# Psy-Fer/SquiggleKit

Hardware: AMD Instinct MI355X
Metric: reads/sec MotifSeq DTW (4k-sample read x 200-sample motif) (higher is better)
Workload: dtype f64 results; u32 fixed-point screening

## Files before the change

### squigglekit_amd/csrc/sk_api.hip

```cpp
#include "sk_common.h"
#include <math.h>
#include <string.h>
#include <stdio.h>
#include <stdlib.h>
#include <vector>

namespace {

int check_i16(const void *sig, int64_t stride, const int32_t *len, int32_t nreads)
{
    if (nreads < 0) return sk_fail(SK_ERR_INVALID, "nreads < 0");
    if (nreads && (!sig || !len)) return sk_fail(SK_ERR_INVALID, "NULL sig/len");
    if (stride <= 0) return sk_fail(SK_ERR_INVALID, "stride must be positive");
    return SK_OK;
}

int check_len_host(const int32_t *len, int32_t nreads, int64_t stride)
{
    for (int32_t r = 0; r < nreads; r++)
        if (len[r] < 0 || (int64_t)len[r] > stride)
            return sk_fail(SK_ERR_INVALID, "len[%d] = %d is outside [0, stride = %lld]", r, len[r], (long long)stride);
    return SK_OK;
}

// ... 42 lines not shown
    cost[0] = fabs(x[0] - y[0]);
    for (int i = 1; i < n; i++) cost[(size_t)i * m] = fabs(x[i] - y[0]) + cost[(size_t)(i - 1) * m];
    for (int j = 1; j < m; j++) cost[j] = fabs(x[0] - y[j]);
    for (int i = 1; i < n; i++) {
        const double *up = cost + (size_t)(i - 1) * m;
        double *row = cost + (size_t)i * m;
        for (int j = 1; j < m; j++) row[j] = fabs(x[i] - y[j]) + cref_min3(up[j], up[j - 1], row[j - 1]);
    }
    const double *last = cost + (size_t)(n - 1) * m;
    int idx = 0;
    double best = last[0];
    if (!(best != best))
        for (int j = 1; j < m; j++) {
            if (last[j] != last[j]) { idx = j; break; }
            if (last[j] < best) { best = last[j]; idx = j; }
        }
    int i = n - 1, j = idx;
    while (i > 0) {
        if (j == 0) { i--; continue; }
        const double up = cost[(size_t)(i - 1) * m + j], dg = cost[(size_t)(i - 1) * m + j - 1], lf = cost[(size_t)i * m + j - 1];
        const double mc = cref_min3(up, dg, lf);
        if (dg == mc)      { i--; j--; }
        else if (lf == mc) { j--; }
        else               { i--; }
    }
    sk_hit h;
    h.dist = last[idx]; h.start = j; h.end = idx; h.n = m; h.flags = 0;
    out[0] = h;
}

struct SubBatches {
    int32_t per = 0, n = 1;
};
SubBatches sub_batches(int32_t nreads, int64_t stride)
{
    SubBatches sb;
    int64_t target = (int64_t)256 << 20;
    if (const char *e = sk_tune("SK_INGEST_MB")) { const long v = atol(e); if (v > 0) target = (int64_t)v << 20; }
    int64_t per = target / (stride * (int64_t)sizeof(int16_t));
    if (per < 4096) per = 4096;
    if (per * 2 > nreads) { sb.per = nreads; sb.n = 1; return sb; }
    sb.n = (int32_t)((nreads + per - 1) / per);
    sb.per = (int32_t)(((int64_t)nreads + sb.n - 1) / sb.n);
    return sb;
}

template <class Step>
int ingest_rows(sk_ctx *c, const SubBatches &B, int16_t *d_rows, const int16_t *sig, int64_t stride, const int32_t *len,
                int32_t nreads, Step step)
{
    int rc;
    if (B.n > 1 && (rc = sk_second_stream(c))) return rc;
    const hipStream_t cs = B.n > 1 ? c->stream2 : c->stream;
    for (int32_t bi = 0; bi < B.n; bi++) {
        const int32_t r0 = bi * B.per;
        const int32_t nr = (nreads - r0 < B.per) ? nreads - r0 : B.per;
        if (nr <= 0) break;
        int16_t *d_sig = d_rows + (size_t)r0 * (size_t)stride;
        int32_t *d_len = (int32_t *)c->len.p + r0;
        SK_HIP(hipMemcpyAsync(d_sig, sig + (size_t)r0 * (size_t)stride, (size_t)nr * (size_t)stride * sizeof(int16_t),
                              hipMemcpyHostToDevice, cs));
        if (len) SK_HIP(hipMemcpyAsync(d_len, len + r0, (size_t)nr * sizeof(int32_t), hipMemcpyHostToDevice, cs));
        if (B.n > 1) {
            SK_HIP(hipEventRecord(c->ev_chunk[bi & 7], cs));
            SK_HIP(hipStreamWaitEvent(c->stream, c->ev_chunk[bi & 7], 0));
        }
        if ((rc = step(r0, nr, d_sig, d_len))) return rc;
    }
    return SK_OK;
}

void redo_forget(sk_ctx *c)
{
    c->redo_route = SK_REDO_NONE;
    c->redo_off.clear();
    c->redo_used = 0;
}

int redo_begin(sk_ctx *c, int32_t nreads, int32_t lists)
{
    redo_forget(c);
    return sk_reserve(c, &c->redo, ((size_t)nreads + 16 * (size_t)lists) * sizeof(int32_t));
}

int redo_list(sk_ctx *c, int route, int32_t nr, int32_t **list)
{
    const size_t end = c->redo_used + (size_t)nr + 16;
    if (end * sizeof(int32_t) > c->redo.cap) return sk_fail(SK_ERR_INVALID, "internal: redo list past its reservation");
    *list = (int32_t *)c->redo.p + c->redo_used;
    c->redo_used = end;
    c->redo_route = route;
    return SK_OK;
}

int redo_count(sk_ctx *c, int route)
{
    if (c->redo_route != route) return -1;
    SK_HIP(hipStreamSynchronize(c->stream));
    int total = 0;
    for (size_t o : c->redo_off) {
        int32_t v = 0;
        SK_HIP(hipMemcpy(&v, (const int32_t *)c->redo.p + o, sizeof v, hipMemcpyDeviceToHost));
        total += v;
    }
    return total;
}
// ... 2388 lines not shown
```

### squigglekit_amd/csrc/sk_common.h

```cpp
#pragma once
#include <hip/hip_runtime.h>
#include <stdint.h>
#include <stddef.h>
#include <stdarg.h>
#include <vector>
#include "squigglekit_hip.h"

#define SK_MAX_DEVICES 16
#define SK_WAVE 64

struct sk_prep {
    int32_t n;
    int32_t flags;
    double  center;
    double  scale;
    double  top;
    double  bot;
};

#define SK_IFLAG_INPLACE 0x100
#define SK_FLAG_PUBLIC   0xff

enum sk_prep_mode { SK_PREP_MEDMAD = 0, SK_PREP_ZSCALE = 1, SK_PREP_SEGMENT = 2, SK_PREP_DRNA = 3 };

enum sk_redo_route { SK_REDO_NONE = 0, SK_REDO_I16 = 1, SK_REDO_F64 = 2, SK_REDO_PA = 3 };

struct sk_buf {
    void  *p = nullptr;
    size_t cap = 0;
};

struct sk_panel_motif {
    int32_t xoff;
    int32_t P;
    int32_t k;
    int32_t pad;
};
struct sk_panel_group {
    int32_t L, R;
    int32_t first, count;
};

struct sk_ctx {
    int         device = -1;
    bool        ready = false;
    hipStream_t stream = nullptr;
    hipStream_t stream2 = nullptr;
    hipStream_t stream3 = nullptr;
    hipEvent_t  ev_r[2] = {nullptr, nullptr};
    hipStream_t stream4 = nullptr;
    hipEvent_t  ev_a = nullptr;
    hipEvent_t  ev_s[2] = {nullptr, nullptr};
    uint32_t    dtw_sparse_calls = 0;
    uint32_t    dtw_audit_calls = 0;
    hipEvent_t  ev_chunk[9] = {};
    hipEvent_t  ev[4] = {nullptr, nullptr, nullptr, nullptr};
    bool        ev_valid = false;
    int         num_cu = 0;
    sk_buf sig;
    sk_buf len;
    sk_buf rlen;
    sk_buf off;
    sk_buf comp;
    sk_buf prep;
    sk_buf mask;
    sk_buf motif;
    sk_buf out;
    sk_buf out2;
    sk_buf misc;
    sk_buf seghints;
    sk_buf pacal;
    sk_buf pull;
    sk_buf pulltext;
    sk_buf sweep;
    sk_buf sweeprec;
    sk_buf hitrows;
    sk_buf bgrec;
    sk_buf pathcnt;
    bool   path_valid = false;
    sk_buf pathlist;
    sk_buf pathscratch;
    sk_buf pathmotif;
    sk_buf pathspans;
    sk_buf events;
    sk_buf poolev;
    sk_buf pool;
    sk_buf panel;
    sk_buf panelwin;
    sk_buf panelaux;
    sk_buf panelrec;
    sk_buf seglev;
    sk_buf seglevwork;
    sk_buf detect;
    sk_buf detectout;
    sk_buf hmm;
    sk_buf hmmpath;
    sk_buf hmmseg;
    std::vector<double> panel_host;
    std::vector<sk_panel_motif> panel_table;
    std::vector<sk_panel_group> panel_groups;
    std::vector<int32_t> panel_long;
    sk_buf ckpt;
    sk_buf motifq;
    sk_buf motif64;
    bool   motif64_valid = false;
    std::vector<double> motif64_host;
    sk_buf lastq;
    sk_buf qflag;
    sk_buf wsoft;
    sk_buf lsum;
    sk_buf wstate;
    sk_buf wrec;
    sk_buf wrecq;
    sk_buf order;
    sk_buf motifw;
    std::vector<double> motifw_host;
    int    motifq_L = 0;
    sk_buf retry;
    sk_buf dtwcnt;
    sk_buf audit;
    sk_buf sib;
    sk_buf sibout;
    sk_buf sibstate;
    bool   retry_dev = false;
    std::vector<unsigned> motifq_host;
    bool   motifq_valid = false;
    sk_buf redo;
    int    redo_route = SK_REDO_NONE;
    std::vector<size_t> redo_off;
    size_t redo_used = 0;
    std::vector<int64_t> pa_off_host;
    int    last_retry = 0;
    std::vector<hipEvent_t> evpool;
    int    prof_chunks = 0;
    int    prof_reads[64] = {0};
    std::vector<double> motif_host;
    std::vector<double> motif_src;
    int    motif_L = 0;
    void  *comm = nullptr;
    sk_buf commbuf;
};

const char *sk_tune(const char *name);

struct sk_entry {
    sk_ctx *c = nullptr;
    sk_entry();
    explicit sk_entry(int slot);
    ~sk_entry();
    sk_entry(const sk_entry &) = delete;
    sk_entry &operator=(const sk_entry &) = delete;
};
#define SK_ENTER(c)                                                                     \
    sk_entry c##_entry_;                                                                \
    sk_ctx *const c = c##_entry_.c;                                                     \
    if (!c) return SK_ERR_NO_DEVICE
sk_ctx *sk_ctx_of(int device);
int  sk_bound_device(void);
int  sk_fail(int code, const char *fmt, ...);
int  sk_reserve(sk_ctx *c, sk_buf *b, size_t bytes);
int  sk_second_stream(sk_ctx *c);
int64_t sk_dtw_chunk_reads(size_t per_read, int64_t nreads);
void    sk_dtw_scratch_shrink(int reset);
#define SK_HIP(call)                                                                    \
    do {                                                                                \
        hipError_t e_ = (call);                                                         \
        if (e_ != hipSuccess)                                                           \
            return sk_fail(SK_ERR_HIP, "%s failed: %s (%s:%d)", #call,                 \
                           hipGetErrorString(e_), __FILE__, __LINE__);                  \
    } while (0)

int sk_launch_prep_i16(sk_ctx *c, const int16_t *d_sig, int64_t stride, const int32_t *d_len,
                       int32_t nreads, int32_t lo, int32_t hi, int mode, double std_scale,
                       int16_t *d_comp, sk_prep *d_prep, uint64_t *d_mask, int64_t mask_stride,
                       int32_t t0 = 0, int32_t t1 = 0x7fffffff,
                       const int32_t *d_list = nullptr, const int32_t *d_count = nullptr,
// ... 197 lines not shown
```

### squigglekit_amd/csrc/sk_runtime.hip

```cpp
#include "sk_common.h"
#include <string>
#include <string.h>
#include <mutex>
#include <stdio.h>
#include <stdlib.h>
#include <string.h>

static thread_local char  g_err[512] = "";
static thread_local int   g_cur = -1;
static sk_ctx             g_ctx[SK_MAX_DEVICES];
static std::mutex         g_mu;
static std::recursive_mutex g_ctx_mu[SK_MAX_DEVICES];

int sk_fail(int code, const char *fmt, ...)
{
    va_list ap;
    va_start(ap, fmt);
    vsnprintf(g_err, sizeof g_err, fmt, ap);
    va_end(ap);
    return code;
}

sk_entry::sk_entry() : sk_entry(g_cur) {}

// ... 9 lines not shown
            return;
        }
        g_ctx_mu[slot].unlock();
    }
    sk_fail(SK_ERR_NO_DEVICE, "no device bound: call sk_init(device) first (no CPU fallback exists)");
}

sk_entry::~sk_entry() { if (c) g_ctx_mu[c - g_ctx].unlock(); }

sk_ctx *sk_ctx_of(int device) { return (device >= 0 && device < SK_MAX_DEVICES) ? &g_ctx[device] : nullptr; }
int sk_bound_device(void) { return g_cur; }

int sk_reserve(sk_ctx *c, sk_buf *b, size_t bytes)
{
    (void)c;
    if (bytes <= b->cap) return SK_OK;
    if (b->p) { SK_HIP(hipFree(b->p)); b->p = nullptr; b->cap = 0; }
    size_t want = bytes + bytes / 8 + 256;
    hipError_t e = hipMalloc(&b->p, want);
    if (e != hipSuccess) {
        b->p = nullptr;
        return sk_fail(SK_ERR_NOMEM, "hipMalloc(%zu) failed: %s", want, hipGetErrorString(e));
    }
    b->cap = want;
    return SK_OK;
}

int sk_second_stream(sk_ctx *c)
{
    if (!c->stream2) {
        SK_HIP(hipStreamCreateWithFlags(&c->stream2, hipStreamNonBlocking));
        for (int i = 0; i < 9; i++) SK_HIP(hipEventCreateWithFlags(&c->ev_chunk[i], hipEventDisableTiming));
    }
    return SK_OK;
}

struct sk_tunable { const char *name, *test_values, *what; };
static const sk_tunable SK_TUNABLES[] = {
    {"SK_DTW_SCHEME",         "full exact2", "DTW scheme: full = one exact pass, exact2 = two exact passes (default: fixed-point screening + certified window)"},
    {"SK_DTW_QL",             "8 16 64",     "lanes per read of the screening scheme (default: by motif length and batch size)"},
    {"SK_DTW_NOFUSE",         "1",           "filter + medmad as their own kernel instead of the screening pass's prologue"},
    {"SK_DTW_FORCE_RETRY_PM", "100 1000",    "per-mille of reads sent through the exact retry whatever the window pass certified (sensitivity runs)"},
    {"SK_DTW_SPAN",           "150 300",     "look-back of the window pass in columns (one tier)"},
    {"SK_DTW_SPAN2",          "0 500",       "look-back of the window pass's second tier (0: none)"},
    {"SK_DTW_CK",             "64 256",      "steps between checkpoints of the screening pass (multiple of 64)"},
    {"SK_DTW_NOSORT",         "1",           "window passes take the reads in file order"},
    {"SK_DTW_SORT_MIN",       "1",           "window passes sort chunks of at least this many reads"},
    {"SK_DTW_NO_EARLY",       "1",           "no early exact retry beside the window passes"},
    {"SK_DTW_NO_SIBLINGS",    "1",           "reads whose candidate columns fall into two clusters take the exact pass (no second window)"},
    {"SK_DTW_NOGUARD",        "1",           "screening scheme without its run-time guard (premise test in the window pass, audit, gated exact fallback): A/B cost runs"},
    {"SK_DTW_AUDIT_PERIOD",   "0 1 64",      "the audit re-runs one read in this many with the exact pass (default 4096; 0: no audit)"},
    {"SK_DTW_HOLE",           "qerr1 fma64 fma64x", "tests: a known precision hole put back (E = 1; the fma sample image for float64 reads, with / without the image-error guard) -- the guard has to notice and the records must not change"},
    {"SK_DTW_SCRATCH_MB",     "8 64",        "checkpoint scratch budget in MB (small values force many chunks)"},
    {"SK_DTW_NO_SMALL",       "1",           "small batches keep the batch lane layout"},
    {"SK_DTW_SMALL_MAX",      "0 100000",    "largest batch that spreads a read over 64 lanes"},
    {"SK_PREP_BLOCK",         "1",           "medmad statistics by the workgroup-per-read kernel"},
    {"SK_PREP_ROUNDS",        "1 3",         "grid rounds of the persistent statistics kernels"},
    {"SK_PREP_PERCU",         "1 2",         "workgroups per CU of the persistent statistics kernels"},
    {"SK_SEG_OLD",            "1",           "segmenter: numpy-order statistics kernels for every read"},
    {"SK_SEG_DELTA_SCALE",    "1e13",        "segmenter: certification margin multiplier (large: every read takes the numpy-order redo)"},
    {"SK_SEG_PA_F64",         "1",           "segmenter, raw reads through the pA conversion: expand to float64 and take the float64 kernels instead of the raw-domain kernel"},
    {"SK_SEG_NO_WG",          "1",           "segmenter, reads of 4 097 .. 65 536 samples: the wavefront-per-read statistics kernel (two looks at a read) instead of the workgroup-per-read one"},
    {"SK_SEG_WG_ALL",         "1",           "segmenter: the workgroup-per-read statistics kernel for every row of 4 097 .. 65 536 samples (default: where it is faster)"},
    {"SK_SEG_OCC",            "7 8",         "segmenter statistics kernel: waves per SIMD the registers are sized for"},
    {"SK_SEG_CHUNKS",         "2 8",         "segmenter: chunks of a large batch (walk of one beside the statistics of the next)"},
    {"SK_WALK_GENERAL",       "1",           "segmenter walk: general step (corrector test live)"},
    {"SK_WALK_SYNC",          "1",           "segmenter walk: run hopping with the 64 lanes of a wavefront on the same word (k_seg_walk3)"},
    {"SK_WALK_OWNPASS",       "1",           "segmenter walk: finds the quiet stretches and anchors in a pass of its own instead of taking the statistics kernel's hints"},
    {"SK_WALK_NOJUMP",        "1",           "segmenter walk: every run is hopped through, no jumps between the stretches of quiet entries"},
    {"SK_WALK_NOWAVE",        "1",           "segmenter walk: a lane per read also for long rows / small batches (no wavefront-per-read walk)"},
    {"SK_WALK_WAVE_MAXREADS", "0 1000000",   "segmenter walk: batches of up to this many reads take the wavefront-per-read walk (default: 16384, 131072 for rows beyond 4 096 samples)"},
    {"SK_DRNA_STEP",          "1",           "dRNA_segmenter, both branches: the per-sample scans instead of the scans by runs / by transitions"},
    {"SK_ROLL_TWO_KERNELS",   "1",           "dRNA_segmenter rolling-mean branch: filter kernel + prefix sums through HBM instead of the one-look kernel (prefix sums in LDS)"},
    {"SK_ROLL_ONE_LOOK",      "1",           "dRNA_segmenter rolling-mean branch: the workgroup-per-read kernel in numpy's order for every read instead of the streaming kernel with certified thresholds"},
    {"SK_ROLL_DELTA_SCALE",   "1e13",        "dRNA_segmenter rolling-mean branch: multiplier of the certification margin (large: every read is redone in numpy's order)"},
    {"SK_HITS_ROW_BYTES",     "1000000",     "hit lists: bytes of the last-row buffer (12 B per column and read; default 2 GiB; small values force many chunks of reads)"},
    {"SK_PANEL_EXACT",        "1",           "motif panel: the one-grid exact kernel also for long windows over many reads (default: those take the screening scheme, one launch set per motif)"},
    {"SK_PATH_LDS_BYTES",     "0",           "alignment paths: bytes of direction words a hit may keep in LDS (default and most 25600; 0: every hit takes the scratch tier)"},
    {"SK_PATH_SCRATCH_BYTES", "1000000",     "alignment paths: byte budget of the scratch tier's slabs (default 1 GiB; small values leave one wavefront)"},
    {"SK_INGEST_MB",          "1 4",         "sub-batch size of the host entry points in MB"},
    {"SK_HMM_SCRATCH_MB",     "1",           "signal HMM state paths: back-pointer scratch budget in MB (default 16384; small values force slices of one 64-read group)"},
    {"SK_F64_OLD",            "1",           "float64 reads: numpy-order statistics kernel for every read"},
    {"SK_F64_LONG_LOOKS",     "1",           "float64 reads of 4 097 .. 40 960 samples: the window-by-window kernel (three to five looks at a read) instead of the workgroup-per-read one (one look)"},
};

const char *sk_tune(const char *name)
{
    const char *on = getenv("SK_TUNING");
    if (!on || on[0] != '1') return nullptr;
    for (const sk_tunable &t : SK_TUNABLES)
        if (strcmp(t.name, name) == 0) return getenv(name);
    return nullptr;
}

static thread_local int g_dtw_shrink = 0;
void sk_dtw_scratch_shrink(int reset) { g_dtw_shrink = reset ? 0 : (g_dtw_shrink < 12 ? g_dtw_shrink + 1 : 12); }

int64_t sk_dtw_chunk_reads(size_t per_read, int64_t nreads)
{
    size_t budget = (size_t)64 << 30;
    int64_t floor_reads = 1024;
    if (const char *e = sk_tune("SK_DTW_SCRATCH_MB")) {
        const long v = atol(e);
        if (v > 0) { budget = (size_t)v << 20; floor_reads = 64; }
    }
    budget >>= g_dtw_shrink;
// ... 24 lines not shown
        sk_fail(SK_ERR_NO_DEVICE, "hipGetDeviceCount: %s", hipGetErrorString(e));
        return 0;
    }
    return n;
}

int sk_init(int device) { return sk_init_slot(device, device); }

int sk_init_slot(int slot, int device)
{
    int n = sk_device_count();
    if (n <= 0) return sk_fail(SK_ERR_NO_DEVICE, "no HIP device visible (this library has no CPU fallback)");
    if (device < 0 || device >= n || device >= SK_MAX_DEVICES)
        return sk_fail(SK_ERR_INVALID, "device %d out of range (0..%d)", device, n - 1);
    if (slot < 0 || slot >= SK_MAX_DEVICES)
        return sk_fail(SK_ERR_INVALID, "context slot %d out of range (0..%d)", slot, SK_MAX_DEVICES - 1);
    std::lock_guard<std::mutex> lk(g_mu);
    sk_ctx *c = &g_ctx[slot];
    std::lock_guard<std::recursive_mutex> c_lock(g_ctx_mu[slot]);
    if (c->ready && c->device != device)
        return sk_fail(SK_ERR_INVALID, "context slot %d already serves device %d", slot, c->device);
    SK_HIP(hipSetDevice(device));
    if (!c->ready) {
        hipDeviceProp_t prop;
        SK_HIP(hipGetDeviceProperties(&prop, device));
        if (strncmp(prop.gcnArchName, "gfx950", 6) != 0)
            return sk_fail(SK_ERR_NO_DEVICE, "device %d is %s; this build targets gfx950 only",
                           device, prop.gcnArchName);
        c->device = device;
        c->num_cu = prop.multiProcessorCount;
        SK_HIP(hipStreamCreateWithFlags(&c->stream, hipStreamNonBlocking));
        for (int i = 0; i < 4; i++) SK_HIP(hipEventCreate(&c->ev[i]));
        c->ready = true;
    }
    g_cur = slot;
    return SK_OK;
}

static void free_buf(sk_buf *b) { if (b->p) (void)hipFree(b->p); b->p = nullptr; b->cap = 0; }

int sk_shutdown(void)
{
    std::lock_guard<std::mutex> lk(g_mu);
    for (int d = 0; d < SK_MAX_DEVICES; d++) {
        sk_ctx *c = &g_ctx[d];
        std::lock_guard<std::recursive_mutex> c_lock(g_ctx_mu[d]);
        if (!c->ready) continue;
        (void)hipSetDevice(c->device);
        (void)hipStreamSynchronize(c->stream);
        sk_buf *bufs[] = {&c->sig, &c->len, &c->off, &c->comp, &c->prep, &c->mask,
                          &c->motif, &c->out, &c->out2, &c->misc, &c->ckpt, &c->retry, &c->motifq, &c->lastq, &c->qflag,
                          &c->motif64, &c->commbuf, &c->dtwcnt, &c->wsoft, &c->wstate, &c->wrec, &c->motifw, &c->lsum, &c->wrecq, &c->order, &c->pacal, &c->seghints, &c->audit, &c->rlen, &c->redo, &c->sib, &c->sibout, &c->sibstate, &c->pull, &c->pulltext, &c->sweep, &c->sweeprec, &c->hitrows, &c->bgrec, &c->pathcnt, &c->pathlist, &c->pathscratch, &c->pathmotif, &c->pathspans, &c->events, &c->poolev, &c->pool, &c->panel, &c->panelwin, &c->panelaux, &c->panelrec, &c->seglev, &c->seglevwork, &c->detect, &c->detectout, &c->hmm, &c->hmmpath, &c->hmmseg};
        for (sk_buf *b : bufs) free_buf(b);
        for (int i = 0; i < 4; i++) (void)hipEventDestroy(c->ev[i]);
        for (hipEvent_t e : c->evpool) (void)hipEventDestroy(e);
        if (c->stream2) {
            (void)hipStreamSynchronize(c->stream2);
            for (int i = 0; i < 9; i++) if (c->ev_chunk[i]) (void)hipEventDestroy(c->ev_chunk[i]);
            (void)hipStreamDestroy(c->stream2);
        }
        if (c->stream3) {
            (void)hipStreamSynchronize(c->stream3);
            for (int i = 0; i < 2; i++) if (c->ev_r[i]) (void)hipEventDestroy(c->ev_r[i]);
            (void)hipStreamDestroy(c->stream3);
        }
        for (int i = 0; i < 2; i++) if (c->ev_s[i]) (void)hipEventDestroy(c->ev_s[i]);
        if (c->stream4) {
            (void)hipStreamSynchronize(c->stream4);
            if (c->ev_a) (void)hipEventDestroy(c->ev_a);
            (void)hipStreamDestroy(c->stream4);
        }
        (void)hipStreamDestroy(c->stream);
        *c = sk_ctx();
    }
    g_cur = -1;
    return SK_OK;
}

int sk_sync(void)
{
    SK_ENTER(c);
    SK_HIP(hipStreamSynchronize(c->stream));
    return SK_OK;
}

int sk_device_name(char *buf, int cap)
{
    SK_ENTER(c);
    if (!buf || cap <= 0) return sk_fail(SK_ERR_INVALID, "bad buffer");
    hipDeviceProp_t prop;
    SK_HIP(hipGetDeviceProperties(&prop, c->device));
    snprintf(buf, (size_t)cap, "%s (%s, %d CUs)", prop.name, prop.gcnArchName, prop.multiProcessorCount);
    return SK_OK;
}

int sk_device_pci_bus_id(char *buf, int cap)
{
    SK_ENTER(c);
    if (!buf || cap < 16) return sk_fail(SK_ERR_INVALID, "bad buffer");
    SK_HIP(hipDeviceGetPCIBusId(buf, cap, c->device));
    return SK_OK;
}

void *sk_dev_alloc(size_t bytes)
{
    sk_entry entry;
// ... 149 lines not shown
```

### squigglekit_amd/csrc/sk_sdtw.hip

```cpp
#include "sk_sdtw_dev.h"
#include <math.h>
#include <stdlib.h>
#include <string.h>
#include <vector>

namespace {

template <int L, int R, int FEED, int MODE>
__global__ __launch_bounds__(256)
void k_sdtw(const sdtw_kargs a)
{
    static_assert(L == 16 || L == 64, "lanes per read");
    constexpr int G = 64 / L;
    constexpr int SHR = (L == 16) ? DPP_ROW_SHR1 : DPP_WAVE_SHR1;
    constexpr int ROL = (L == 16) ? DPP_ROW_ROL1 : DPP_WAVE_ROL1;
    constexpr bool TRACK = (MODE != MODE_DIST);
    constexpr int CKW = R + 3;
    const double INF = __builtin_huge_val();

    const int lane = threadIdx.x & 63;
    const int wave = blockIdx.x * (blockDim.x >> 6) + (threadIdx.x >> 6);
    const int g = lane / L, l = lane % L;
    int slot = wave * G + g;
    int nreads = a.nreads;
// ... 580 lines not shown
    int32_t *alist = nullptr;  sk_hit *aout = nullptr;
    if (naudit) {
        if ((rc = sk_reserve(c, &c->audit, ((size_t)naudit + 2) * sizeof(int32_t) + 16 + (size_t)naudit * sizeof(sk_hit)))) return rc;
        alist = (int32_t *)c->audit.p;
        aout = (sk_hit *)((char *)c->audit.p + ((((size_t)naudit + 2) * sizeof(int32_t) + 15) & ~(size_t)15));
    }
    auto launch_audit = [&](hipStream_t stream) -> int {
        if (!naudit) return SK_OK;
        sk_audit_pick(alist, naudit, audit_period, a->nreads, c->dtw_audit_calls++, stream ? stream : c->stream);
        SK_HIP(hipGetLastError());
        sdtw_kargs kr = k;
        kr.read0 = 0; kr.ridx = alist + 2; kr.count_ptr = alist; kr.ckpt = nullptr; kr.out = aout; kr.out_by_slot = 1;
        kr.total_ptr = guard + SK_GUARD_AUDITED; kr.list_off = 0;
        const int R64 = (N + 63) / 64, P64 = 64 * R64 - N;
        sdtw_fn f64 = (L == 16) ? pick_any(a->feed, 64, R64, MODE_FULL) : nullptr;
        if (f64) {
            sdtw_kargs k64 = kr;
            k64.xlay = (const double *)c->motif64.p; k64.P = P64;
            k64.nreads = naudit < 8192 ? naudit : 8192;
            int rc2;
            if ((rc2 = launch(c, f64, k64, 64, stream))) return rc2;
            if (naudit <= 8192) return SK_OK;
            kr.list_off = 8192; kr.total_ptr = nullptr; kr.nreads = naudit - 8192;
            return launch(c, ff, kr, L, stream);
        }
        kr.nreads = naudit;
        return launch(c, ff, kr, L, stream);
    };
    auto finish_guard = [&]() -> int {
        if (!guarded) return SK_OK;
        if (naudit) {
            sk_audit_compare(alist, aout, a->out, naudit, guard, c->stream);
            SK_HIP(hipGetLastError());
        }
        sdtw_kargs kf = k;
        kf.read0 = 0; kf.nreads = a->nreads; kf.ridx = nullptr; kf.count_ptr = nullptr; kf.ckpt = nullptr;
        kf.gate_ptr = guard + SK_GUARD_ALARM; kf.guard = guard;
        return launch(c, ff, kf, L);
    };
    if (qok) {
        const bool early = sk_tune("SK_DTW_NO_EARLY") == nullptr;
        if (early && !c->stream3) {
            SK_HIP(hipStreamCreateWithFlags(&c->stream3, hipStreamNonBlocking));
            for (int i = 0; i < 2; i++) SK_HIP(hipEventCreateWithFlags(&c->ev_r[i], hipEventDisableTiming));
        }
        if (early && naudit && !c->stream4) {
            SK_HIP(hipStreamCreateWithFlags(&c->stream4, hipStreamNonBlocking));
            SK_HIP(hipEventCreateWithFlags(&c->ev_a, hipEventDisableTiming));
        }
        if ((rc = sk_launch_sdtw_screen(c, a, ck, span_q, span2, cnt, cnt + 2, early ? ecnt : nullptr,
                                        early ? ecnt + 2 : nullptr))) return rc;
        if (early) {
            SK_HIP(hipStreamWaitEvent(c->stream3, c->ev_r[0], 0));
            if ((rc = launch_retry(ecnt, c->stream3))) return rc;
            SK_HIP(hipEventRecord(c->ev_r[1], c->stream3));
            if (naudit) {
                SK_HIP(hipStreamWaitEvent(c->stream4, c->ev_r[0], 0));
                if ((rc = launch_audit(c->stream4))) return rc;
                SK_HIP(hipEventRecord(c->ev_a, c->stream4));
            }
        }
        if ((rc = launch_retry())) return rc;
        if (early) {
            SK_HIP(hipStreamWaitEvent(c->stream, c->ev_r[1], 0));
            if (naudit) SK_HIP(hipStreamWaitEvent(c->stream, c->ev_a, 0));
        } else if ((rc = launch_audit(nullptr))) return rc;
        if ((rc = finish_guard())) return rc;
        SK_HIP(hipEventRecord(c->ev[3], c->stream));
        return SK_OK;
    }
    const int nck = (int)((maxlen + L - 1) / ck);
    const size_t per_read = (size_t)(nck > 0 ? nck : 1) * L * (R + 3) * sizeof(double);
    int64_t chunk;
    while (true) {
        chunk = sk_dtw_chunk_reads(per_read, a->nreads);
        rc = sk_reserve(c, &c->ckpt, (size_t)chunk * per_read);
        if (rc != SK_ERR_NOMEM || chunk <= 1024) break;
        sk_dtw_scratch_shrink(0);
    }
    if (rc) return rc;
    k.ckpt = (double *)c->ckpt.p; k.nck = nck; k.ck = ck; k.span = span;
    k.retry = cnt + 2; k.retry_cnt = cnt;
    const size_t nchunks = (size_t)((a->nreads + chunk - 1) / chunk);
    while (c->evpool.size() < 3 * nchunks) {
        hipEvent_t e;
        SK_HIP(hipEventCreate(&e));
        c->evpool.push_back(e);
    }
    c->prof_chunks = 0;
    for (int64_t r0 = 0; r0 < a->nreads; r0 += chunk) {
        k.read0 = (int)r0;
        k.nreads = (int)((a->nreads - r0 < chunk) ? a->nreads - r0 : chunk);
        hipEvent_t *ev = &c->evpool[3 * (size_t)c->prof_chunks];
        SK_HIP(hipEventRecord(ev[0], c->stream));
        if ((rc = launch(c, fa, k, L))) return rc;
        SK_HIP(hipEventRecord(ev[1], c->stream));
        if ((rc = launch(c, fb, k, L))) return rc;
        SK_HIP(hipEventRecord(ev[2], c->stream));
        c->prof_reads[c->prof_chunks < 64 ? c->prof_chunks : 63] = k.nreads;
        c->prof_chunks++;
    }
    if ((rc = launch_retry())) return rc;
    SK_HIP(hipEventRecord(c->ev[3], c->stream));
    return SK_OK;
}
```

### squigglekit_amd/csrc/sk_sdtwq.hip

```cpp
#include "sk_sdtw_dev.h"
#include "sk_prepw_dev.h"
#include <math.h>
#include <stdlib.h>
#include <string.h>
#include <vector>

#ifndef SK_SDTWQ_FEED
#define SK_SDTWQ_FEED 0
#define SK_SDTWQ_MAIN 1
#endif

namespace {

template <int R>
__device__ __forceinline__ void qcolumn(const unsigned (&old)[R], unsigned (&nw)[R], const unsigned (&xq)[R],
                                        unsigned yq, unsigned dg, unsigned up)
{
    constexpr int R4 = R & ~3;
#pragma unroll
    for (int k = 0; k < R4; k += 4) {
        asm("v_min3_u32 %0, %12, %4, %13\n\t"
            "v_sad_u32 %0, %8, %14, %0 clamp\n\t"
            "v_min3_u32 %1, %4, %5, %0\n\t"
            "v_sad_u32 %1, %9, %14, %1 clamp\n\t"
// ... 829 lines not shown
    const int s = blockIdx.x * blockDim.x + threadIdx.x;
    if (s == 0 && nsib_total) atomicAdd(nsib_total, min(*cnt, cap));
    if (s >= min(*cnt, cap)) return;
    const int r = sib[s].r;
    sk_hit A = out[r];
    const sk_hit B = so[s];
    if (A.start < 0) return;
    if (B.n == 1) {
        if (B.dist < A.dist) { A.dist = B.dist; A.start = B.start; A.end = B.end; out[r] = A; }
    } else {
        A.dist = __builtin_nan(""); A.start = -1; A.end = -1;
        out[r] = A;
        retry[atomicAdd(retry_cnt, 1)] = r;
    }
}

int sk_launch_sdtw_screen(sk_ctx *c, const sk_sdtw_args *a, int ck, int span, int span2,
                          int32_t *d_retry_cnt, int32_t *d_retry, int32_t *d_early_cnt, int32_t *d_early)
{
    const int N = a->nmotif;
    int L, R;
    screen_layout(N, a->nreads, a->max_len, &L, &R);
    const int P = L * R - N;
    int rc;
    if (!c->motifq_valid || c->motifq_L != L) {
        SK_HIP(hipStreamSynchronize(c->stream));
        std::vector<unsigned> &layq = c->motifq_host;
        std::vector<double> &layw = c->motifw_host;
        layq.assign((size_t)L * R, 0x80000000u);
        layw.assign((size_t)L * R, 0.0);
        int row = 0;
        for (int l = 0; l < L; l++) {
            const int cnt = (l < P) ? R - 1 : R;
            for (int k = 0; k < cnt; k++, row++) {
                layq[(size_t)l * R + k] = (unsigned)((int)rint(a->motif[row] * QSCALE)) + 0x80000000u;
                layw[(size_t)l * R + k] = a->motif[row];
            }
        }
        if ((rc = sk_reserve(c, &c->motifq, layq.size() * sizeof(unsigned)))) return rc;
        if ((rc = sk_reserve(c, &c->motifw, layw.size() * sizeof(double)))) return rc;
        SK_HIP(hipMemcpyAsync(c->motifq.p, layq.data(), layq.size() * sizeof(unsigned), hipMemcpyHostToDevice, c->stream));
        SK_HIP(hipMemcpyAsync(c->motifw.p, layw.data(), layw.size() * sizeof(double), hipMemcpyHostToDevice, c->stream));
        c->motifq_valid = true;
        c->motifq_L = L;
    }

    const int64_t maxlen = a->max_len;
    const int nck = (int)((maxlen + L - 1) / ck);
    const size_t lq_stride = (size_t)((maxlen + 3 * L + 7) & ~(int64_t)3);
    const size_t state_bytes = (size_t)L * (R + 2) * sizeof(unsigned);
    const size_t ck_bytes = (size_t)L * ((R + 3) / 2) * sizeof(unsigned);
    const size_t per_read = (size_t)(nck > 0 ? nck : 1) * ck_bytes + lq_stride * sizeof(unsigned) + state_bytes +
                            (size_t)(nck + 1) * L * sizeof(unsigned) + 64;
    int64_t chunk;
    while (true) {
        chunk = sk_dtw_chunk_reads(per_read, a->nreads);
        rc = sk_reserve(c, &c->ckpt, (size_t)chunk * (size_t)(nck > 0 ? nck : 1) * ck_bytes);
        if (!rc) rc = sk_reserve(c, &c->lastq, (size_t)chunk * lq_stride * sizeof(unsigned));
        if (!rc) rc = sk_reserve(c, &c->wstate, (size_t)chunk * state_bytes);
        if (!rc) rc = sk_reserve(c, &c->lsum, (size_t)chunk * (size_t)(nck + 1) * L * sizeof(unsigned));
        if (rc != SK_ERR_NOMEM || chunk <= 1024) break;
        sk_dtw_scratch_shrink(0);
    }
    if (rc) return rc;
    if ((rc = sk_reserve(c, &c->qflag, (size_t)chunk * sizeof(int32_t)))) return rc;
    if ((rc = sk_reserve(c, &c->wrec, (size_t)chunk * sizeof(wrec)))) return rc;
    if ((rc = sk_reserve(c, &c->wrecq, (size_t)chunk * sizeof(wrec)))) return rc;
    int sort_min = 32768;
    if (const char *e = sk_tune("SK_DTW_SORT_MIN")) { const int v = atoi(e); if (v > 0) sort_min = v; }
    const bool sorted = chunk >= sort_min && sk_tune("SK_DTW_NOSORT") == nullptr;
    if (sorted && (rc = sk_reserve(c, &c->order, ((size_t)chunk + ORDER_BINS) * sizeof(int32_t)))) return rc;
    const bool tiers = span2 > span;
    if (tiers && (rc = sk_reserve(c, &c->wsoft, ((size_t)chunk + 1) * sizeof(int32_t)))) return rc;
    const bool siblings = sk_tune("SK_DTW_NO_SIBLINGS") == nullptr;
    const int sib_cap = (int)(chunk / 64 + 1024);
    if (siblings) {
        if ((rc = sk_reserve(c, &c->sib, 16 + (size_t)sib_cap * sizeof(sibrec)))) return rc;
        if ((rc = sk_reserve(c, &c->sibout, (size_t)sib_cap * sizeof(sk_hit)))) return rc;
        if ((rc = sk_reserve(c, &c->sibstate, (size_t)sib_cap * (state_bytes + sizeof(wrec))))) return rc;
        if (c->stream3 && !c->ev_s[0])
            for (int i = 0; i < 2; i++) SK_HIP(hipEventCreateWithFlags(&c->ev_s[i], hipEventDisableTiming));
    }

    typedef void *(*pick_fn)(int, int, int);
    const pick_fn pk = a->feed == SK_FEED_I16 ? (pick_fn)sk_sdtwq_pick_feed0
                     : a->feed == SK_FEED_F64_NORM ? (pick_fn)sk_sdtwq_pick_feed1 : (pick_fn)sk_sdtwq_pick_feed2;
    sdtw_fn fq = (sdtw_fn)pk(P == 0 ? 3 : 0, L, R), fp = (sdtw_fn)pk(1, L, R), fw = (sdtw_fn)pk(2, L, R);
    if (!fq || !fp || !fw) return sk_fail(SK_ERR_UNSUPPORTED, "no screening kernel for L=%d R=%d", L, R);

    sdtw_kargs k;
    memset(&k, 0, sizeof k);
    k.samples = a->samples; k.samples_raw = a->samples_raw; k.stride = a->stride; k.off = a->off; k.prep = a->prep;
    k.xlay = (const double *)c->motifw.p; k.xlayq = (const unsigned *)c->motifq.p; k.P = P; k.out = a->out;
    k.nck = nck; k.ck = ck; k.span = span; k.retry = d_retry; k.retry_cnt = d_retry_cnt;
    k.ckq = (unsigned *)c->ckpt.p; k.lastq = (unsigned *)c->lastq.p; k.lq_stride = (int64_t)lq_stride;
    k.qflag = (int32_t *)c->qflag.p; k.lsum = (unsigned *)c->lsum.p;
    k.wstate = (unsigned *)c->wstate.p; k.wrec = c->wrec.p; k.wrec_q = c->wrecq.p;
    k.early_cnt = d_early_cnt; k.early = d_early;
    k.qerr = (unsigned)(N + maxlen + 2);
    k.wmax = 4 * ck;
    k.lds_wave_words = (64 / L) * ck;
    k.guard = sk_tune("SK_DTW_NOGUARD") ? nullptr : (int32_t *)c->dtwcnt.p + 8;
    k.wsteps = (unsigned long long *)((char *)c->dtwcnt.p + 64);
    if (const char *e = sk_tune("SK_DTW_HOLE")) {
        k.hole = strcmp(e, "qerr1") == 0 ? SK_HOLE_QERR1 : strcmp(e, "fma64") == 0 ? SK_HOLE_FMA64
               : strcmp(e, "fma64x") == 0 ? SK_HOLE_FMA64_UNGUARDED : SK_HOLE_NONE;
        if (k.hole == SK_HOLE_QERR1) k.qerr = 1;
    }
    if (const char *e = sk_tune("SK_DTW_FORCE_RETRY_PM")) {
        const int pm = atoi(e);
        if (pm > 0) k.force_retry = pm >= 1000 ? 1024 : (pm * 1024 + 999) / 1000;
    }

    size_t fz_lds = 0;
    const sk_prep_fuse fz = a->fuse ? *a->fuse : sk_prep_fuse();
    if (a->fuse) {
        const int need = fz.mode == SK_PREP_ZSCALE ? (int)((a->stride * 2 + 15) / 16 * 4) : (((fz.hi - fz.lo - 1) + 3) & ~3);
        if (need > k.lds_wave_words) k.lds_wave_words = need;
    }
    fz_lds = (size_t)4 * (size_t)k.lds_wave_words * sizeof(unsigned);
    if (fz_lds + 5 * 1024 > 64 * 1024)
        return sk_fail(SK_ERR_INVALID, "SK_DTW_CK=%d with %d lanes per read needs %zu bytes of LDS per workgroup (limit 65536): "
                       "use a smaller multiple of 64", ck, L, fz_lds + 5 * 1024);

    const size_t nchunks = (size_t)((a->nreads + chunk - 1) / chunk);
    while (c->evpool.size() < 3 * nchunks) {
        hipEvent_t e;
        SK_HIP(hipEventCreate(&e));
        c->evpool.push_back(e);
    }
    c->prof_chunks = 0;
    const int reads_per_block = 4 * (64 / L);
    for (int64_t r0 = 0; r0 < a->nreads; r0 += chunk) {
        k.read0 = (int)r0;
        k.nreads = (int)((a->nreads - r0 < chunk) ? a->nreads - r0 : chunk);
        const int grid = (k.nreads + reads_per_block - 1) / reads_per_block;
        if (a->fuse) {
            k.fz_raw = fz.raw; k.fz_len = fz.len; k.fz_lo = fz.lo; k.fz_hi = fz.hi;
            k.fz_mode = fz.mode == SK_PREP_ZSCALE ? 1 : 0;
            k.fz_vec = ((((uintptr_t)fz.raw & 15) == 0 && (a->stride % 8) == 0) ? 1 : 0) |
                       ((((uintptr_t)a->samples & 15) == 0 && (a->stride % 8) == 0) ? 2 : 0);
        }
        hipEvent_t *ev = &c->evpool[3 * (size_t)c->prof_chunks];
        k.sib = nullptr; k.sib_cnt = nullptr; k.sib_out = nullptr; k.tier2 = 0;
        if (siblings) {
            SK_HIP(hipMemsetAsync(c->sib.p, 0, 16, c->stream));
            k.sib_cnt = (int32_t *)c->sib.p; k.sib = (char *)c->sib.p + 16; k.sib_out = (sk_hit *)c->sibout.p;
            k.sib_cap = sib_cap;
        }
        SK_HIP(hipEventRecord(ev[0], c->stream));
        k.clk = (r0 == 0) ? (unsigned long long *)((char *)c->dtwcnt.p + 16) : nullptr;
        hipLaunchKernelGGL(fq, dim3(grid), dim3(256), fz_lds, c->stream, k);
        k.fz_raw = nullptr;
        if (d_early_cnt && r0 + chunk >= a->nreads) SK_HIP(hipEventRecord(c->ev_r[0], c->stream));
        SK_HIP(hipGetLastError());
        if (siblings) {
            sdtw_kargs ks = k;
            ks.tier2 = 2; ks.wl_list = nullptr; ks.wl_count = k.sib_cnt; ks.soft = nullptr; ks.soft_cnt = nullptr;
            ks.span = tiers ? span2 : span; ks.total_ptr = nullptr; ks.nreads = sib_cap;
            ks.wstate = (unsigned *)c->sibstate.p; ks.wrec = (char *)c->sibstate.p + (size_t)sib_cap * state_bytes;
            const int sgrid = (sib_cap + reads_per_block - 1) / reads_per_block;
            hipStream_t ss = c->stream3 ? c->stream3 : c->stream;
            if (c->stream3) {
                SK_HIP(hipEventRecord(c->ev_s[0], c->stream));
                SK_HIP(hipStreamWaitEvent(c->stream3, c->ev_s[0], 0));
            }
            hipLaunchKernelGGL(fp, dim3(sgrid), dim3(256), 0, ss, ks);
            hipLaunchKernelGGL(fw, dim3(sgrid), dim3(256), 0, ss, ks);
            SK_HIP(hipGetLastError());
            if (c->stream3) SK_HIP(hipEventRecord(c->ev_s[1], c->stream3));
        }
        SK_HIP(hipEventRecord(ev[1], c->stream));
        const int32_t *order = nullptr;
        if (sorted && k.nreads >= sort_min) {
            order_args oa;
            oa.rec = (const wrec *)c->wrecq.p; oa.qflag = (const int32_t *)c->qflag.p;
            oa.nreads = k.nreads; oa.read0 = k.read0; oa.span = span; oa.ck = ck; oa.nck = nck; oa.L = L; oa.wmax = k.wmax;
            oa.hist = (int32_t *)c->order.p; oa.order = oa.hist + ORDER_BINS;
            SK_HIP(hipMemsetAsync(oa.hist, 0, ORDER_BINS * sizeof(int32_t), c->stream));
            const int og = (k.nreads + ORDER_TPB * ORDER_IPT - 1) / (ORDER_TPB * ORDER_IPT);
            hipLaunchKernelGGL(k_order_count, dim3(og), dim3(ORDER_TPB), 0, c->stream, oa);
            hipLaunchKernelGGL(k_order_scan, dim3(1), dim3(ORDER_BINS), 0, c->stream, oa.hist);
            hipLaunchKernelGGL(k_order_scatter, dim3(og), dim3(ORDER_TPB), 0, c->stream, oa);
            SK_HIP(hipGetLastError());
            order = oa.order;
        }
        k.tier2 = 0;
        if (tiers) {
            int32_t *soft = (int32_t *)c->wsoft.p;
            SK_HIP(hipMemsetAsync(soft, 0, sizeof(int32_t), c->stream));
            k.span = span; k.wl_list = order; k.wl_count = nullptr; k.soft = soft + 1; k.soft_cnt = soft;
            hipLaunchKernelGGL(fp, dim3(grid), dim3(256), 0, c->stream, k);
            hipLaunchKernelGGL(fw, dim3(grid), dim3(256), 0, c->stream, k);
            SK_HIP(hipGetLastError());
            k.span = span2; k.wl_list = soft + 1; k.wl_count = soft; k.soft = nullptr; k.soft_cnt = nullptr;
            k.tier2 = 1;
            k.total_ptr = (int32_t *)c->dtwcnt.p + 1;
        } else {
            k.wl_list = order; k.wl_count = nullptr;
        }
        hipLaunchKernelGGL(fp, dim3(grid), dim3(256), 0, c->stream, k);
        k.total_ptr = nullptr;
        hipLaunchKernelGGL(fw, dim3(grid), dim3(256), 0, c->stream, k);
        SK_HIP(hipGetLastError());
        if (siblings) {
            if (c->stream3) SK_HIP(hipStreamWaitEvent(c->stream, c->ev_s[1], 0));
            hipLaunchKernelGGL(k_sib_combine, dim3((sib_cap + 255) / 256), dim3(256), 0, c->stream,
                               (const sibrec *)k.sib, (const int32_t *)k.sib_cnt, sib_cap, (const sk_hit *)k.sib_out, k.out,
                               d_retry, d_retry_cnt, (int32_t *)c->dtwcnt.p + 8 + 6);
            SK_HIP(hipGetLastError());
        }
        SK_HIP(hipEventRecord(ev[2], c->stream));
        c->prof_reads[c->prof_chunks < 64 ? c->prof_chunks : 63] = k.nreads;
        c->prof_chunks++;
    }
    return SK_OK;
}
#endif
```

Before: 16.82 million.

## Split screening DTW launch set across two stream lanes with separate scratch

```diff
diff --git a/squigglekit_amd/csrc/sk_api.hip b/squigglekit_amd/csrc/sk_api.hip
--- a/squigglekit_amd/csrc/sk_api.hip
+++ b/squigglekit_amd/csrc/sk_api.hip
@@ -118,6 +118,8 @@
     int rc;
     if (B.n > 1 && (rc = sk_second_stream(c))) return rc;
     const hipStream_t cs = B.n > 1 ? c->stream2 : c->stream;
+    struct Owns { sk_ctx *c; bool was; ~Owns() { c->stream2_copies = was; } } owns = {c, c->stream2_copies};
+    if (B.n > 1) c->stream2_copies = true;
     for (int32_t bi = 0; bi < B.n; bi++) {
         const int32_t r0 = bi * B.per;
         const int32_t nr = (nreads - r0 < B.per) ? nreads - r0 : B.per;
diff --git a/squigglekit_amd/csrc/sk_common.h b/squigglekit_amd/csrc/sk_common.h
--- a/squigglekit_amd/csrc/sk_common.h
+++ b/squigglekit_amd/csrc/sk_common.h
@@ -39,6 +39,14 @@
 struct sk_panel_group {
     int32_t L, R;
     int32_t first, count;
+};
+
+struct sk_dtw_lane {
+    sk_buf ckpt, lastq, wstate, lsum, qflag, wrec, wrecq, order, wsoft, sib, sibout, sibstate;
+    hipEvent_t ev_s[2] = {nullptr, nullptr};
+    hipEvent_t ev_fork = nullptr;
+    hipEvent_t ev_q = nullptr;
+    hipEvent_t ev_join = nullptr;
 };
 
 struct sk_ctx {
@@ -122,6 +130,9 @@
     sk_buf sib;
     sk_buf sibout;
     sk_buf sibstate;
+    sk_dtw_lane lane1;
+    bool   lane1_q = false;
+    bool   stream2_copies = false;
     bool   retry_dev = false;
     std::vector<unsigned> motifq_host;
     bool   motifq_valid = false;
diff --git a/squigglekit_amd/csrc/sk_runtime.hip b/squigglekit_amd/csrc/sk_runtime.hip
--- a/squigglekit_amd/csrc/sk_runtime.hip
+++ b/squigglekit_amd/csrc/sk_runtime.hip
@@ -85,6 +85,8 @@
     {"SK_DTW_AUDIT_PERIOD",   "0 1 64",      "the audit re-runs one read in this many with the exact pass (default 4096; 0: no audit)"},
     {"SK_DTW_HOLE",           "qerr1 fma64 fma64x", "tests: a known precision hole put back (E = 1; the fma sample image for float64 reads, with / without the image-error guard) -- the guard has to notice and the records must not change"},
     {"SK_DTW_SCRATCH_MB",     "8 64",        "checkpoint scratch budget in MB (small values force many chunks)"},
+    {"SK_DTW_SPLIT",          "1 2 3",       "pieces wanted per screening launch set; they alternate between two lanes (streams with scratch of their own), so one piece's window passes run beside the other's screening sweep (1: one lane, one piece per scratch chunk)"},
+    {"SK_DTW_SPLIT_MIN",      "64 1000",     "fewest reads a piece of a split launch set may hold (default 131072)"},
     {"SK_DTW_NO_SMALL",       "1",           "small batches keep the batch lane layout"},
     {"SK_DTW_SMALL_MAX",      "0 100000",    "largest batch that spreads a read over 64 lanes"},
     {"SK_PREP_BLOCK",         "1",           "medmad statistics by the workgroup-per-read kernel"},
@@ -215,6 +217,11 @@
                           &c->motif, &c->out, &c->out2, &c->misc, &c->ckpt, &c->retry, &c->motifq, &c->lastq, &c->qflag,
                           &c->motif64, &c->commbuf, &c->dtwcnt, &c->wsoft, &c->wstate, &c->wrec, &c->motifw, &c->lsum, &c->wrecq, &c->order, &c->pacal, &c->seghints, &c->audit, &c->rlen, &c->redo, &c->sib, &c->sibout, &c->sibstate, &c->pull, &c->pulltext, &c->sweep, &c->sweeprec, &c->hitrows, &c->bgrec, &c->pathcnt, &c->pathlist, &c->pathscratch, &c->pathmotif, &c->pathspans, &c->events, &c->poolev, &c->pool, &c->panel, &c->panelwin, &c->panelaux, &c->panelrec, &c->seglev, &c->seglevwork, &c->detect, &c->detectout, &c->hmm, &c->hmmpath, &c->hmmseg};
         for (sk_buf *b : bufs) free_buf(b);
+        sk_dtw_lane &l1 = c->lane1;
+        sk_buf *bufs1[] = {&l1.ckpt, &l1.lastq, &l1.wstate, &l1.lsum, &l1.qflag, &l1.wrec, &l1.wrecq, &l1.order, &l1.wsoft,
+                           &l1.sib, &l1.sibout, &l1.sibstate};
+        for (sk_buf *b : bufs1) free_buf(b);
+        for (hipEvent_t e : {l1.ev_s[0], l1.ev_s[1], l1.ev_fork, l1.ev_q, l1.ev_join}) if (e) (void)hipEventDestroy(e);
         for (int i = 0; i < 4; i++) (void)hipEventDestroy(c->ev[i]);
         for (hipEvent_t e : c->evpool) (void)hipEventDestroy(e);
         if (c->stream2) {
diff --git a/squigglekit_amd/csrc/sk_sdtw.hip b/squigglekit_amd/csrc/sk_sdtw.hip
--- a/squigglekit_amd/csrc/sk_sdtw.hip
+++ b/squigglekit_amd/csrc/sk_sdtw.hip
@@ -656,10 +656,12 @@
                                         early ? ecnt + 2 : nullptr))) return rc;
         if (early) {
             SK_HIP(hipStreamWaitEvent(c->stream3, c->ev_r[0], 0));
+            if (c->lane1_q) SK_HIP(hipStreamWaitEvent(c->stream3, c->lane1.ev_q, 0));
             if ((rc = launch_retry(ecnt, c->stream3))) return rc;
             SK_HIP(hipEventRecord(c->ev_r[1], c->stream3));
             if (naudit) {
                 SK_HIP(hipStreamWaitEvent(c->stream4, c->ev_r[0], 0));
+                if (c->lane1_q) SK_HIP(hipStreamWaitEvent(c->stream4, c->lane1.ev_q, 0));
                 if ((rc = launch_audit(c->stream4))) return rc;
                 SK_HIP(hipEventRecord(c->ev_a, c->stream4));
             }
diff --git a/squigglekit_amd/csrc/sk_sdtwq.hip b/squigglekit_amd/csrc/sk_sdtwq.hip
--- a/squigglekit_amd/csrc/sk_sdtwq.hip
+++ b/squigglekit_amd/csrc/sk_sdtwq.hip
@@ -905,34 +905,70 @@
     const size_t ck_bytes = (size_t)L * ((R + 3) / 2) * sizeof(unsigned);
     const size_t per_read = (size_t)(nck > 0 ? nck : 1) * ck_bytes + lq_stride * sizeof(unsigned) + state_bytes +
                             (size_t)(nck + 1) * L * sizeof(unsigned) + 64;
+    const int reads_per_block = 4 * (64 / L);
+    int split = 2;
+    int64_t split_min = 131072;
+    if (const char *e = sk_tune("SK_DTW_SPLIT")) { const int v = atoi(e); if (v >= 1) split = v; }
+    if (const char *e = sk_tune("SK_DTW_SPLIT_MIN")) { const long v = atol(e); if (v >= 1) split_min = v; }
+    if ((int64_t)split > a->nreads / split_min) split = (int)(a->nreads / split_min);
+    if (split < 1 || c->stream2_copies) split = 1;
+    const int nlanes = split > 1 ? 2 : 1;
+    if (nlanes == 2 && (rc = sk_second_stream(c))) return rc;
+    struct lane_t {
+        hipStream_t stream;
+        sk_buf *ckpt, *lastq, *wstate, *lsum, *qflag, *wrec, *wrecq, *order, *wsoft, *sib, *sibout, *sibstate;
+        hipEvent_t *ev_s;
+    };
+    sk_dtw_lane &l1 = c->lane1;
+    lane_t lanes[2] = {
+        {c->stream, &c->ckpt, &c->lastq, &c->wstate, &c->lsum, &c->qflag, &c->wrec, &c->wrecq, &c->order, &c->wsoft,
+         &c->sib, &c->sibout, &c->sibstate, c->ev_s},
+        {c->stream2, &l1.ckpt, &l1.lastq, &l1.wstate, &l1.lsum, &l1.qflag, &l1.wrec, &l1.wrecq, &l1.order, &l1.wsoft,
+         &l1.sib, &l1.sibout, &l1.sibstate, l1.ev_s}};
     int64_t chunk;
     while (true) {
-        chunk = sk_dtw_chunk_reads(per_read, a->nreads);
-        rc = sk_reserve(c, &c->ckpt, (size_t)chunk * (size_t)(nck > 0 ? nck : 1) * ck_bytes);
-        if (!rc) rc = sk_reserve(c, &c->lastq, (size_t)chunk * lq_stride * sizeof(unsigned));
-        if (!rc) rc = sk_reserve(c, &c->wstate, (size_t)chunk * state_bytes);
-        if (!rc) rc = sk_reserve(c, &c->lsum, (size_t)chunk * (size_t)(nck + 1) * L * sizeof(unsigned));
+        chunk = sk_dtw_chunk_reads(per_read * (size_t)nlanes, a->nreads);
+        if (split > 1) {
+            int64_t piece = (a->nreads + split - 1) / split;
+            piece = (piece + reads_per_block - 1) / reads_per_block * reads_per_block;
+            if (piece < chunk) chunk = piece;
+        }
+        rc = SK_OK;
+        for (int ln = 0; ln < nlanes && !rc; ln++) {
+            rc = sk_reserve(c, lanes[ln].ckpt, (size_t)chunk * (size_t)(nck > 0 ? nck : 1) * ck_bytes);
+            if (!rc) rc = sk_reserve(c, lanes[ln].lastq, (size_t)chunk * lq_stride * sizeof(unsigned));
+            if (!rc) rc = sk_reserve(c, lanes[ln].wstate, (size_t)chunk * state_bytes);
+            if (!rc) rc = sk_reserve(c, lanes[ln].lsum, (size_t)chunk * (size_t)(nck + 1) * L * sizeof(unsigned));
+        }
         if (rc != SK_ERR_NOMEM || chunk <= 1024) break;
         sk_dtw_scratch_shrink(0);
     }
     if (rc) return rc;
-    if ((rc = sk_reserve(c, &c->qflag, (size_t)chunk * sizeof(int32_t)))) return rc;
-    if ((rc = sk_reserve(c, &c->wrec, (size_t)chunk * sizeof(wrec)))) return rc;
-    if ((rc = sk_reserve(c, &c->wrecq, (size_t)chunk * sizeof(wrec)))) return rc;
     int sort_min = 32768;
     if (const char *e = sk_tune("SK_DTW_SORT_MIN")) { const int v = atoi(e); if (v > 0) sort_min = v; }
     const bool sorted = chunk >= sort_min && sk_tune("SK_DTW_NOSORT") == nullptr;
-    if (sorted && (rc = sk_reserve(c, &c->order, ((size_t)chunk + ORDER_BINS) * sizeof(int32_t)))) return rc;
     const bool tiers = span2 > span;
-    if (tiers && (rc = sk_reserve(c, &c->wsoft, ((size_t)chunk + 1) * sizeof(int32_t)))) return rc;
     const bool siblings = sk_tune("SK_DTW_NO_SIBLINGS") == nullptr;
     const int sib_cap = (int)(chunk / 64 + 1024);
-    if (siblings) {
-        if ((rc = sk_reserve(c, &c->sib, 16 + (size_t)sib_cap * sizeof(sibrec)))) return rc;
-        if ((rc = sk_reserve(c, &c->sibout, (size_t)sib_cap * sizeof(sk_hit)))) return rc;
-        if ((rc = sk_reserve(c, &c->sibstate, (size_t)sib_cap * (state_bytes + sizeof(wrec))))) return rc;
-        if (c->stream3 && !c->ev_s[0])
-            for (int i = 0; i < 2; i++) SK_HIP(hipEventCreateWithFlags(&c->ev_s[i], hipEventDisableTiming));
+    for (int ln = 0; ln < nlanes; ln++) {
+        const lane_t &ls = lanes[ln];
+        if ((rc = sk_reserve(c, ls.qflag, (size_t)chunk * sizeof(int32_t)))) return rc;
+        if ((rc = sk_reserve(c, ls.wrec, (size_t)chunk * sizeof(wrec)))) return rc;
+        if ((rc = sk_reserve(c, ls.wrecq, (size_t)chunk * sizeof(wrec)))) return rc;
+        if (sorted && (rc = sk_reserve(c, ls.order, ((size_t)chunk + ORDER_BINS) * sizeof(int32_t)))) return rc;
+        if (tiers && (rc = sk_reserve(c, ls.wsoft, ((size_t)chunk + 1) * sizeof(int32_t)))) return rc;
+        if (siblings) {
+            if ((rc = sk_reserve(c, ls.sib, 16 + (size_t)sib_cap * sizeof(sibrec)))) return rc;
+            if ((rc = sk_reserve(c, ls.sibout, (size_t)sib_cap * sizeof(sk_hit)))) return rc;
+            if ((rc = sk_reserve(c, ls.sibstate, (size_t)sib_cap * (state_bytes + sizeof(wrec))))) return rc;
+            if (c->stream3 && !ls.ev_s[0])
+                for (int i = 0; i < 2; i++) SK_HIP(hipEventCreateWithFlags(&ls.ev_s[i], hipEventDisableTiming));
+        }
+    }
+    if (nlanes == 2 && !l1.ev_fork) {
+        SK_HIP(hipEventCreateWithFlags(&l1.ev_fork, hipEventDisableTiming));
+        SK_HIP(hipEventCreateWithFlags(&l1.ev_q, hipEventDisableTiming));
+        SK_HIP(hipEventCreateWithFlags(&l1.ev_join, hipEventDisableTiming));
     }
 
     typedef void *(*pick_fn)(int, int, int);
@@ -946,9 +982,7 @@
     k.samples = a->samples; k.samples_raw = a->samples_raw; k.stride = a->stride; k.off = a->off; k.prep = a->prep;
     k.xlay = (const double *)c->motifw.p; k.xlayq = (const unsigned *)c->motifq.p; k.P = P; k.out = a->out;
     k.nck = nck; k.ck = ck; k.span = span; k.retry = d_retry; k.retry_cnt = d_retry_cnt;
-    k.ckq = (unsigned *)c->ckpt.p; k.lastq = (unsigned *)c->lastq.p; k.lq_stride = (int64_t)lq_stride;
-    k.qflag = (int32_t *)c->qflag.p; k.lsum = (unsigned *)c->lsum.p;
-    k.wstate = (unsigned *)c->wstate.p; k.wrec = c->wrec.p; k.wrec_q = c->wrecq.p;
+    k.lq_stride = (int64_t)lq_stride;
     k.early_cnt = d_early_cnt; k.early = d_early;
     k.qerr = (unsigned)(N + maxlen + 2);
     k.wmax = 4 * ck;
@@ -983,8 +1017,21 @@
         c->evpool.push_back(e);
     }
     c->prof_chunks = 0;
-    const int reads_per_block = 4 * (64 / L);
-    for (int64_t r0 = 0; r0 < a->nreads; r0 += chunk) {
+    c->lane1_q = false;
+    if (nlanes == 2) {
+        SK_HIP(hipEventRecord(l1.ev_fork, c->stream));
+        SK_HIP(hipStreamWaitEvent(c->stream2, l1.ev_fork, 0));
+    }
+    const int64_t npieces = (int64_t)nchunks;
+    int64_t piece = 0;
+    for (int64_t r0 = 0; r0 < a->nreads; r0 += chunk, piece++) {
+        const int ln = nlanes == 2 ? (int)(piece & 1) : 0;
+        const lane_t &ls = lanes[ln];
+        const hipStream_t st = ls.stream;
+        k.ckq = (unsigned *)ls.ckpt->p; k.lastq = (unsigned *)ls.lastq->p;
+        k.qflag = (int32_t *)ls.qflag->p; k.lsum = (unsigned *)ls.lsum->p;
+        k.wstate = (unsigned *)ls.wstate->p; k.wrec = ls.wrec->p; k.wrec_q = ls.wrecq->p;
+        k.span = span; k.wl_list = nullptr; k.wl_count = nullptr; k.soft = nullptr; k.soft_cnt = nullptr;
         k.read0 = (int)r0;
         k.nreads = (int)((a->nreads - r0 < chunk) ? a->nreads - r0 : chunk);
         const int grid = (k.nreads + reads_per_block - 1) / reads_per_block;
@@ -997,54 +1044,57 @@
         hipEvent_t *ev = &c->evpool[3 * (size_t)c->prof_chunks];
         k.sib = nullptr; k.sib_cnt = nullptr; k.sib_out = nullptr; k.tier2 = 0;
         if (siblings) {
-            SK_HIP(hipMemsetAsync(c->sib.p, 0, 16, c->stream));
-            k.sib_cnt = (int32_t *)c->sib.p; k.sib = (char *)c->sib.p + 16; k.sib_out = (sk_hit *)c->sibout.p;
+            SK_HIP(hipMemsetAsync(ls.sib->p, 0, 16, st));
+            k.sib_cnt = (int32_t *)ls.sib->p; k.sib = (char *)ls.sib->p + 16; k.sib_out = (sk_hit *)ls.sibout->p;
             k.sib_cap = sib_cap;
         }
-        SK_HIP(hipEventRecord(ev[0], c->stream));
+        SK_HIP(hipEventRecord(ev[0], st));
         k.clk = (r0 == 0) ? (unsigned long long *)((char *)c->dtwcnt.p + 16) : nullptr;
-        hipLaunchKernelGGL(fq, dim3(grid), dim3(256), fz_lds, c->stream, k);
+        hipLaunchKernelGGL(fq, dim3(grid), dim3(256), fz_lds, st, k);
         k.fz_raw = nullptr;
-        if (d_early_cnt && r0 + chunk >= a->nreads) SK_HIP(hipEventRecord(c->ev_r[0], c->stream));
+        if (d_early_cnt && piece + nlanes >= npieces) {
+            SK_HIP(hipEventRecord(ln ? l1.ev_q : c->ev_r[0], st));
+            if (ln) c->lane1_q = true;
+        }
         SK_HIP(hipGetLastError());
         if (siblings) {
             sdtw_kargs ks = k;
             ks.tier2 = 2; ks.wl_list = nullptr; ks.wl_count = k.sib_cnt; ks.soft = nullptr; ks.soft_cnt = nullptr;
             ks.span = tiers ? span2 : span; ks.total_ptr = nullptr; ks.nreads = sib_cap;
-            ks.wstate = (unsigned *)c->sibstate.p; ks.wrec = (char *)c->sibstate.p + (size_t)sib_cap * state_bytes;
+            ks.wstate = (unsigned *)ls.sibstate->p; ks.wrec = (char *)ls.sibstate->p + (size_t)sib_cap * state_bytes;
             const int sgrid = (sib_cap + reads_per_block - 1) / reads_per_block;
-            hipStream_t ss = c->stream3 ? c->stream3 : c->stream;
+            hipStream_t ss = c->stream3 ? c->stream3 : st;
             if (c->stream3) {
-                SK_HIP(hipEventRecord(c->ev_s[0], c->stream));
-                SK_HIP(hipStreamWaitEvent(c->stream3, c->ev_s[0], 0));
+                SK_HIP(hipEventRecord(ls.ev_s[0], st));
+                SK_HIP(hipStreamWaitEvent(c->stream3, ls.ev_s[0], 0));
             }
             hipLaunchKernelGGL(fp, dim3(sgrid), dim3(256), 0, ss, ks);
             hipLaunchKernelGGL(fw, dim3(sgrid), dim3(256), 0, ss, ks);
             SK_HIP(hipGetLastError());
-            if (c->stream3) SK_HIP(hipEventRecord(c->ev_s[1], c->stream3));
-        }
-        SK_HIP(hipEventRecord(ev[1], c->stream));
+            if (c->stream3) SK_HIP(hipEventRecord(ls.ev_s[1], c->stream3));
+        }
+        SK_HIP(hipEventRecord(ev[1], st));
         const int32_t *order = nullptr;
         if (sorted && k.nreads >= sort_min) {
             order_args oa;
-            oa.rec = (const wrec *)c->wrecq.p; oa.qflag = (const int32_t *)c->qflag.p;
+            oa.rec = (const wrec *)ls.wrecq->p; oa.qflag = (const int32_t *)ls.qflag->p;
             oa.nreads = k.nreads; oa.read0 = k.read0; oa.span = span; oa.ck = ck; oa.nck = nck; oa.L = L; oa.wmax = k.wmax;
-            oa.hist = (int32_t *)c->order.p; oa.order = oa.hist + ORDER_BINS;
-            SK_HIP(hipMemsetAsync(oa.hist, 0, ORDER_BINS * sizeof(int32_t), c->stream));
+            oa.hist = (int32_t *)ls.order->p; oa.order = oa.hist + ORDER_BINS;
+            SK_HIP(hipMemsetAsync(oa.hist, 0, ORDER_BINS * sizeof(int32_t), st));
             const int og = (k.nreads + ORDER_TPB * ORDER_IPT - 1) / (ORDER_TPB * ORDER_IPT);
-            hipLaunchKernelGGL(k_order_count, dim3(og), dim3(ORDER_TPB), 0, c->stream, oa);
-            hipLaunchKernelGGL(k_order_scan, dim3(1), dim3(ORDER_BINS), 0, c->stream, oa.hist);
-            hipLaunchKernelGGL(k_order_scatter, dim3(og), dim3(ORDER_TPB), 0, c->stream, oa);
+            hipLaunchKernelGGL(k_order_count, dim3(og), dim3(ORDER_TPB), 0, st, oa);
+            hipLaunchKernelGGL(k_order_scan, dim3(1), dim3(ORDER_BINS), 0, st, oa.hist);
+            hipLaunchKernelGGL(k_order_scatter, dim3(og), dim3(ORDER_TPB), 0, st, oa);
             SK_HIP(hipGetLastError());
             order = oa.order;
         }
         k.tier2 = 0;
         if (tiers) {
-            int32_t *soft = (int32_t *)c->wsoft.p;
-            SK_HIP(hipMemsetAsync(soft, 0, sizeof(int32_t), c->stream));
+            int32_t *soft = (int32_t *)ls.wsoft->p;
+            SK_HIP(hipMemsetAsync(soft, 0, sizeof(int32_t), st));
             k.span = span; k.wl_list = order; k.wl_count = nullptr; k.soft = soft + 1; k.soft_cnt = soft;
-            hipLaunchKernelGGL(fp, dim3(grid), dim3(256), 0, c->stream, k);
-            hipLaunchKernelGGL(fw, dim3(grid), dim3(256), 0, c->stream, k);
+            hipLaunchKernelGGL(fp, dim3(grid), dim3(256), 0, st, k);
+            hipLaunchKernelGGL(fw, dim3(grid), dim3(256), 0, st, k);
             SK_HIP(hipGetLastError());
             k.span = span2; k.wl_list = soft + 1; k.wl_count = soft; k.soft = nullptr; k.soft_cnt = nullptr;
             k.tier2 = 1;
@@ -1052,21 +1102,25 @@
         } else {
             k.wl_list = order; k.wl_count = nullptr;
         }
-        hipLaunchKernelGGL(fp, dim3(grid), dim3(256), 0, c->stream, k);
+        hipLaunchKernelGGL(fp, dim3(grid), dim3(256), 0, st, k);
         k.total_ptr = nullptr;
-        hipLaunchKernelGGL(fw, dim3(grid), dim3(256), 0, c->stream, k);
+        hipLaunchKernelGGL(fw, dim3(grid), dim3(256), 0, st, k);
         SK_HIP(hipGetLastError());
         if (siblings) {
-            if (c->stream3) SK_HIP(hipStreamWaitEvent(c->stream, c->ev_s[1], 0));
-            hipLaunchKernelGGL(k_sib_combine, dim3((sib_cap + 255) / 256), dim3(256), 0, c->stream,
+            if (c->stream3) SK_HIP(hipStreamWaitEvent(st, ls.ev_s[1], 0));
+            hipLaunchKernelGGL(k_sib_combine, dim3((sib_cap + 255) / 256), dim3(256), 0, st,
                                (const sibrec *)k.sib, (const int32_t *)k.sib_cnt, sib_cap, (const sk_hit *)k.sib_out, k.out,
                                d_retry, d_retry_cnt, (int32_t *)c->dtwcnt.p + 8 + 6);
             SK_HIP(hipGetLastError());
         }
-        SK_HIP(hipEventRecord(ev[2], c->stream));
+        SK_HIP(hipEventRecord(ev[2], st));
         c->prof_reads[c->prof_chunks < 64 ? c->prof_chunks : 63] = k.nreads;
         c->prof_chunks++;
     }
+    if (nlanes == 2) {
+        SK_HIP(hipEventRecord(l1.ev_join, c->stream2));
+        SK_HIP(hipStreamWaitEvent(c->stream, l1.ev_join, 0));
+    }
     return SK_OK;
 }
 #endif
```

Result: no change. 16.67 million (-0.9%).
